# octavian-ganea/equidock_public

Measured on AMD Instinct MI355X. Metric: protein-pairs/sec (fwd+bwd) per IEGMN stack, higher is better.
Workload: dtype f32; 1 GPU; B: DB5.5-sized batch of 8 pairs x (200,200) residues, k=10, 8-layer IEGMN hdim 64, 50 heads, fp32; pairs_per_gpu=8, nodes_per_gpu=3200, edges_per_gpu=32000, layers=8, parallelism=dp1, weights=PyTorch default init (seed 0), ROT key/query x40 (SURVEY.md section 8c), svd_guard_pairs=0, launch_mode=hipGraph replay

## Files before the change

equidock_public_amd/_lib.py:

```python
import ctypes as C
import os

import torch

HERE = os.path.dirname(os.path.abspath(__file__))
LIB_PATH = os.path.join(HERE, 'libequidock_hip.so')
if os.environ.get('EQD_EXP_LIBRARY'):
    LIB_PATH = os.environ['EQD_EXP_LIBRARY']

EQD_MAX_SRC = 6
ABI_VERSION = 9
PARAMS_PER_LAYER = 19
GLOBAL_PARAMS = 5

c_float_p = C.POINTER(C.c_float)
c_int_p = C.POINTER(C.c_int32)


class EqdGraph(C.Structure):
    _fields_ = [('n_pairs', C.c_int32), ('n_lig', C.c_int32), ('n_rec', C.c_int32), ('n_nodes', C.c_int32),
                ('n_edges', C.c_int32), ('n_tiles', C.c_int32), ('n_att_items', C.c_int32), ('max_seg', C.c_int32),
                ('seg_off', C.c_void_p), ('src', C.c_void_p), ('dst', C.c_void_p), ('rowptr', C.c_void_p),
                ('csc_ptr', C.c_void_p), ('csc_eid', C.c_void_p), ('tile_node', C.c_void_p),
                ('att_items', C.c_void_p), ('res_id', C.c_void_p), ('mu_r_norm', C.c_void_p), ('he', C.c_void_p),
# ... 60 lines not shown
                ('dln_b', C.c_void_p), ('dW2', C.c_void_p), ('db2', C.c_void_p), ('dWc1', C.c_void_p),
                ('dbc1', C.c_void_p), ('dwc2', C.c_void_p), ('dbc2', C.c_void_p)]


_lib = None
_is_sim = False
profiling = False


class EquidockHipError(RuntimeError):
    pass


def _declare(lib):
    lib.eqd_abi_version.restype = C.c_int
    lib.eqd_last_error.restype = C.c_char_p
    lib.eqd_tile_edges.restype = C.c_int
    lib.eqd_is_simulator.restype = C.c_int
    lib.eqd_model_saved_bytes.restype = C.c_size_t
    lib.eqd_model_scratch_bytes.restype = C.c_size_t
    lib.eqd_atb_partial_bytes.restype = C.c_size_t
    lib.eqd_edge_message_bwd_workspace_bytes.restype = C.c_size_t
    lib.eqd_keypoint_pool_bwd_workspace_bytes.restype = C.c_size_t
    lib.eqd_clash_workspace_bytes.restype = C.c_size_t
    lib.eqd_node_update_bwd_workspace_bytes.restype = C.c_size_t
    lib.eqd_cross_attention_bwd_ds_workspace_bytes.restype = C.c_size_t
    lib.eqd_profile_name.restype = C.c_char_p
    lib.eqd_profile_us.restype = C.c_float
    lib.eqd_tunables_reload.restype = None
    for name in ('eqd_model_layer_state', 'eqd_model_lrelu_signs', 'eqd_model_head_backward', 'eqd_profile_begin', 'eqd_profile_end', 'eqd_profile_mark', 'eqd_ctx_create', 'eqd_ctx_destroy', 'eqd_model_check', 'eqd_model_forward', 'eqd_model_backward', 'eqd_linear', 'eqd_atb',
                 'eqd_edge_message_fwd', 'eqd_edge_message_bwd', 'eqd_edge_message_bwd_kernel_only',
                 'eqd_cross_attention_fwd', 'eqd_cross_attention_fwd_bf16', 'eqd_cross_attention_bwd_bf16',
                 'eqd_cross_attention_bwd', 'eqd_cross_attention_bwd_ds',
           'eqd_keypoint_pool_fwd', 'eqd_keypoint_pool_bwd', 'eqd_kabsch_fwd', 'eqd_kabsch_bwd',
                 'eqd_rigid_apply_fwd', 'eqd_rigid_apply_bwd', 'eqd_pair_losses_fwd', 'eqd_pair_losses_bwd', 'eqd_scalar_loss', 'eqd_pocket_ot_cost',
                 'eqd_pocket_ot_fwd', 'eqd_pocket_ot_bwd', 'eqd_rigid_augment', 'eqd_protein_graph_distances',
                 'eqd_protein_graph_select', 'eqd_protein_graph_edges', 'eqd_clash_iterations', 'eqd_dropout_pack_edges', 'eqd_dropout_draw',
                 'eqd_node_update_fwd', 'eqd_node_update_bwd', 'eqd_selftest_lane_exchanges'):
        getattr(lib, name).restype = C.c_int


EXPORTS = ('eqd_model_layer_state', 'eqd_model_lrelu_signs', 'eqd_model_head_backward', 'eqd_profile_begin', 'eqd_profile_end', 'eqd_profile_mark', 'eqd_profile_name', 'eqd_profile_us', 'eqd_ctx_create', 'eqd_ctx_destroy', 'eqd_abi_version', 'eqd_last_error', 'eqd_tile_edges', 'eqd_is_simulator', 'eqd_model_saved_bytes', 'eqd_model_saved_layout',
           'eqd_model_scratch_bytes', 'eqd_model_check', 'eqd_model_forward', 'eqd_model_backward', 'eqd_linear',
           'eqd_atb_partial_bytes', 'eqd_atb', 'eqd_edge_message_fwd', 'eqd_edge_message_bwd_workspace_bytes',
           'eqd_edge_message_bwd', 'eqd_edge_message_bwd_kernel_only', 'eqd_cross_attention_fwd',
           'eqd_cross_attention_bwd', 'eqd_cross_attention_bwd_ds', 'eqd_cross_attention_bwd_ds_workspace_bytes', 'eqd_cross_attention_fwd_bf16', 'eqd_cross_attention_bwd_bf16',
           'eqd_keypoint_pool_fwd', 'eqd_keypoint_pool_bwd',
           'eqd_keypoint_pool_bwd_workspace_bytes',
           'eqd_kabsch_fwd', 'eqd_kabsch_bwd', 'eqd_rigid_apply_fwd', 'eqd_rigid_apply_bwd', 'eqd_pair_losses_fwd',
           'eqd_pair_losses_bwd', 'eqd_scalar_loss', 'eqd_pocket_ot_cost', 'eqd_pocket_ot_fwd', 'eqd_pocket_ot_bwd',
           'eqd_rigid_augment', 'eqd_protein_graph_distances', 'eqd_protein_graph_select', 'eqd_protein_graph_edges',
           'eqd_clash_workspace_bytes', 'eqd_clash_iterations', 'eqd_dropout_pack_edges', 'eqd_dropout_draw',
           'eqd_tunables_reload', 'eqd_node_update_fwd', 'eqd_node_update_bwd_workspace_bytes', 'eqd_node_update_bwd',
           'eqd_selftest_lane_exchanges', 'eqd_chain_resident_proj_launches', 'eqd_selftest_node_chain_fwd', 'eqd_model_node_state')


def load_library():
    global _lib, _is_sim
    if _lib is not None:
        return _lib
    if not os.path.exists(LIB_PATH):
        raise EquidockHipError(
            f"{LIB_PATH} is missing: build it with `python -m equidock_public_amd.build` (hipcc, gfx950). "
            "There is no CPU fallback for the IEGMN hot path.")
    lib = C.CDLL(LIB_PATH)
    _declare(lib)
    if lib.eqd_abi_version() != ABI_VERSION:
        raise EquidockHipError(f"ABI version mismatch: library {lib.eqd_abi_version()} != {ABI_VERSION}")
    _lib, _is_sim = lib, bool(lib.eqd_is_simulator())
    return _lib


def load_library_for_testing(path):
    global _lib, _is_sim
    lib = C.CDLL(path)
    _declare(lib)
    _lib, _is_sim = lib, bool(lib.eqd_is_simulator())
    return _lib


def unload_for_testing():
    global _lib, _is_sim
    _lib, _is_sim = None, False


tunables_generation = 0


def reload_tunables():
    global tunables_generation
    tunables_generation += 1
    if _lib is not None:
        _lib.eqd_tunables_reload()


def is_simulator():
    return _is_sim


def check(rc):
    if rc != 0:
        raise EquidockHipError(f"libequidock_hip error {rc}: {_lib.eqd_last_error().decode()}")


def require_device(t, what='tensor'):
    if _is_sim:
        if t.is_cuda:
# ... 62 lines not shown
```

equidock_public_amd/csrc/eqd_common.h:

```cpp
#pragma once
#include <hip/hip_runtime.h>
#include <stdint.h>

#include "../../include/equidock_hip.h"

typedef float f32x4 __attribute__((ext_vector_type(4)));
typedef unsigned int u32x4 __attribute__((ext_vector_type(4)));

#define EQD_BLOCK 256
#define EQD_WAVES 4
#define EQD_NEG_BIG (-1.0e30f)

__device__ __forceinline__ f32x4 mfma4(float a, float b, f32x4 c) {
    return __builtin_amdgcn_mfma_f32_16x16x4f32(a, b, c, 0, 0, 0);
}
#ifdef EQD_TRACE
extern __device__ long long eqd_trace_buf[1024];
#define EQD_TR(slot)                                                                          \
    do {                                                                                      \
        const int trs_ = (slot);                                                              \
        if (blockIdx.x == 0 && blockIdx.y == 0 && threadIdx.x == 0 && trs_ < 256) {           \
            eqd_trace_buf[2 * trs_] = clock64();                                              \
            eqd_trace_buf[2 * trs_ + 1] = wall_clock64();                                     \
        }                                                                                     \
// ... 319 lines not shown

struct EqdArena {
    char* base;
    size_t size, off;
    bool ok;
    EqdArena(void* p, size_t n) : base((char*)p), size(n), off(0), ok(true) {}
    template <typename T>
    T* take(size_t count) {
        size_t bytes = eqd_align_up(count * sizeof(T));
        if (base == nullptr || off + bytes > size) {
            ok = false;
            off += bytes;
            return nullptr;
        }
        T* r = (T*)(base + off);
        off += bytes;
        return r;
    }
};

#define EQD_RED_MAXSEG 64
struct EqdRedSeg {
    const float* partial;
    int nparts, pstride, n;
    float* out;
    int cols, cols_valid, ld_out;
};
struct EqdRedArg {
    EqdRedSeg s[EQD_RED_MAXSEG];
    int chain_first[EQD_RED_MAXSEG], chain_len[EQD_RED_MAXSEG];
    int chain_blk0[EQD_RED_MAXSEG];
    int nchains;
};
int eqd_launch_reduce_segments(const EqdRedSeg* segs, int nseg, hipStream_t st);
struct EqdRedList {
    EqdRedSeg seg[512];
    int n;
};

#define EQD_CHAIN_MAXJOBS 8
struct EqdChainJob {
    EqdLinJob lin;
    int src_local[EQD_MAX_SRC];
    int out_local;
    int type;
    float* aux;
    int prefetch_next;
    int next_lin;
};
struct EqdChainArg {
    EqdChainJob j[EQD_CHAIN_MAXJOBS];
    int njobs;
};
int eqd_launch_rowchain(const EqdChainJob* jobs, int njobs, int rows, hipStream_t st, int* partial_rows = nullptr);
size_t eqd_atb_batch_partial_bytes(int rows);
int eqd_atb_tail_wanted(const EqdLinJob* dh0_job, int n_atb_jobs);
int eqd_atb_with_tail(const EqdAtbJob* jobs, int njobs, void* partial, size_t partial_bytes, hipStream_t st,
                      const EqdLinJob* dh0_job, const EqdGraph* g, const float* dh0acc, const float* dh0b, int ld, int d_emb,
                      float* demb, float* emb_partial, EqdRedList* defer);
int eqd_rows_resident(int rows);
int eqd_rowres80_on();
int eqd_chain_carries_proj(int rows);
int eqd_row_tiles(int rows);
int eqd_rowchain_blocks(int rows);

int eqd_launch_vec_reduce(const float* partial, int nparts, int pstride, int n, float* out, hipStream_t st);
int eqd_launch_embed_fwd(const EqdGraph* g, const float* emb, int d_emb, int use_mu, float* h0, int ld, hipStream_t st);
struct EqdRedList;
int eqd_launch_embed_bwd(const EqdGraph* g, const float* dh0, const float* dh0b, int ld, int d_emb, float* demb,
                         float* partial, hipStream_t st, EqdRedList* defer = nullptr);
size_t eqd_embed_bwd_partial_floats(const EqdGraph* g, int d_emb);
struct EqdGatherCall {
    const float *dz, *dxrel, *d_xnew;
    float a;
    float *dP, *dQ, *dx;
    int dz_bf16;
};
struct EqdGatherArgs;
int eqd_gather_plan(const EqdGraph* g, const EqdGatherCall* c, EqdRedList* pending, EqdGatherArgs* GA, EqdRedArg* RA, int* nblk);
int eqd_gather_rest(EqdRedList* pending, hipStream_t st);
int eqd_attention_bwd_gather_fused(const EqdGraph* g, int d, const float* q, const float* k, const float* v, const float* out,
                                   const float* d_out, bool bf16);
int eqd_attention_ds_stride(const EqdGraph* g);
size_t eqd_attention_ds_bytes(const EqdGraph* g);
int eqd_attention_ds_wanted(const EqdGraph* g, int d, bool bf16);
int eqd_launch_seg_start(const EqdGraph* g, int32_t* seg_start, hipStream_t st);
int eqd_attention_fwd_bf16_impl(const EqdGraph* g, int d, const float* q, const float* k, const float* v, float* out,
                                float* lse, hipStream_t stream, bool qkv_bf16);
int eqd_launch_attention_bwd_gather(const EqdGraph* g, int d, const float* q, const float* k, const float* v, const float* out,
                                    const float* lse, const float* d_out, float* dq, float* dk, float* dv, float* delta,
                                    float qk_slope, bool bf16, const EqdGatherCall* gc, EqdRedList* pending, hipStream_t st,
                                    float* ds = nullptr, const int32_t* seg_start = nullptr, bool qkv_bf16 = false);
int eqd_launch_node_gather(const EqdGraph* g, const float* dz, const float* dxrel, const float* d_xnew, float a,
                           float* dP, float* dQ, float* dx, hipStream_t st, EqdRedList* pending = nullptr,
                           bool dz_bf16 = false);
int eqd_launch_ln_act_bwd(const float* y_act, const float* d_out, const float* gamma, int rows, int d, int ld,
                          float slope, float eps, float* dz, float* dgamma, float* dbeta, float* partial,
                          hipStream_t st, EqdRedList* defer = nullptr);
int eqd_edge_message_bwd_impl(const EqdGraph* g, const EqdEdgeParams* p, const float* P, const float* Q, const float* x,
                              const float* d_aggr_msg, const float* d_xnew, float* dP, float* dQ, float* dx,
                              const EqdEdgeGrads* grads, void* workspace, size_t ws_bytes, hipStream_t st,
                              float* part_override, EqdRedList* defer, EqdGatherCall* hold_gather = nullptr);
size_t eqd_edge_bwd_vecp_floats(const EqdGraph* g);
int eqd_edge_attn_fwd(const EqdGraph* g, const EqdEdgeParams* p, const float* P, const float* Q, const float* x,
                      float* aggr_msg, float* x_new, int d_att, const float* q, const float* k, const float* v,
                      float* att_out, float* lse, hipStream_t st);
int eqd_keypoint_pool_fwd_impl(const EqdGraph* g, int n_heads, const float* Wk, const float* Wq, const float* qmean,
// ... 27 lines not shown
```

equidock_public_amd/csrc/eqd_driver.hip:

```cpp
#include "eqd_common.h"

#include <vector>

#include <string.h>

namespace {

enum {
    P_W1 = 0, P_B1, P_LNG, P_LNB, P_W2, P_B2, P_WQ, P_WK, P_WV, P_WN1, P_BN1, P_NLG, P_NLB, P_WN2, P_BN2,
    P_WC1, P_BC1, P_WC2, P_BC2
};
enum { G_EMB = 0, G_WK, G_WQ, G_WM, G_BM };

struct Dims {
    int N, E, B, K, L, d0, dh;
    int d_in(int l) const { return l == 0 ? d0 : dh; }
    int d_att(int l) const { return (d_in(l) + 15) / 16 * 16; }
    int ldw1(int l) const { return 2 * d_in(l) + 27 + 15; }
    int ldwn(int l) const { return d0 + 2 * d_in(l) + dh; }
};

Dims make_dims(const EqdModelDesc* m, const EqdGraph* g) {
    Dims D;
    D.N = g->n_nodes; D.E = g->n_edges; D.B = g->n_pairs; D.K = m->n_heads; D.L = m->n_layers;
// ... 794 lines not shown
            for (int i = 0; i < nj; ++i) jobs[i] = cj[i].lin;
            RC(eqd_linear(jobs, nj, st));
        }
        hipStream_t sat = (cx && m->cross_msgs) ? cx->sa : st;
        if (sat != st) {
            HIPOK(hipEventRecord(cx->fork, st));
            HIPOK(hipStreamWaitEvent(sat, cx->fork, 0));
        }
        EqdEdgeParams ep = edge_params(D, m, l, p, drop);
        ep.aggr_bf16 = Ls.aggr_b;
        ep.xh_save = Ls.xh_e; ep.rstd_save = Ls.rstd_e; ep.zpos_save = Ls.zpos_e;
        if (m->cross_msgs && sat == st && !m->storage_bf16) {
            RC(eqd_edge_attn_fwd(g, &ep, Ls.P, Ls.Q, S.x[l], Ls.aggr_msg, S.x[l + 1], da, Ls.qa, Ls.ka, Ls.va, Ls.aggr_cross,
                                 Ls.lse, st));
        } else {
            if (m->cross_msgs) {
                if (m->storage_bf16 && Ls.qa_b)
                    RC(eqd_attention_fwd_bf16_impl(g, da, (const float*)Ls.qa_b, (const float*)Ls.ka_b, (const float*)Ls.va_b,
                                                   Ls.aggr_cross, Ls.lse, sat, true));
                else if (m->storage_bf16)
                    RC(eqd_cross_attention_fwd_bf16(g, da, Ls.qa, Ls.ka, Ls.va, Ls.aggr_cross, Ls.lse, sat));
                else
                    RC(eqd_cross_attention_fwd(g, da, Ls.qa, Ls.ka, Ls.va, Ls.aggr_cross, Ls.lse, sat));
            } else {
                if (hipMemsetAsync(Ls.aggr_cross, 0, (size_t)N * da * sizeof(float), st) != hipSuccess) return EQD_ERR_LAUNCH;
            }
            if (sat != st) HIPOK(hipEventRecord(cx->join_a, sat));
            RC(eqd_edge_message_fwd(g, &ep, Ls.P, Ls.Q, S.x[l], Ls.aggr_msg, S.x[l + 1], st));
            if (sat != st) HIPOK(hipStreamWaitEvent(st, cx->join_a, 0));
        }
        NodeFwdChain fc;
        fc.N = N; fc.d = d; fc.da = da; fc.d0 = D.d0; fc.dh = D.dh; fc.ldn = D.ldwn(l); fc.ld_a1n = Ls.ld_a1n;
        fc.slope = slope; fc.eps = eps; fc.skip = m->skip_weight_h;
        fc.h = h; fc.aggr_msg = Ls.aggr_msg; fc.aggr_cross = Ls.aggr_cross; fc.h0 = S.h[0];
        fc.Wn1 = p[P_WN1]; fc.Bn1 = p[P_BN1]; fc.ln_g = p[P_NLG]; fc.ln_b = p[P_NLB]; fc.Wn2 = p[P_WN2]; fc.Bn2 = p[P_BN2];
        fc.drop_mul = drop_node(D, drop, l);
        fc.a1n = Ls.a1n; fc.y_act = Ls.y_act; fc.h_out = S.h[l + 1]; fc.a1n_b = Ls.a1n_b; fc.hb_out = S.hb[l + 1];
        fc.next = nullptr; fc.head = nullptr;
        const bool carry_small = d == 64 && D.dh == 64 && D.d0 > 64 && D.d0 <= 80 && da == 64 && m->cross_msgs &&
                                 !m->storage_bf16 && eqd_chain_carries_proj(N);
        proj_in_chain = l + 1 < D.L && D.d_in(l + 1) == 64 && D.dh == 64 && 2 + (m->cross_msgs ? 5 : 2) <= EQD_CHAIN_MAXJOBS &&
                        (((d == 64 || (m->storage_bf16 && eqd_rowres80_on())) && eqd_rows_resident(N)) ||
                         (carry_small && D.d_att(l + 1) == 64));
        head_in_chain = l + 1 == D.L && carry_small;
        NodePre np;
        if (proj_in_chain) {
            np = node_pre(l + 1);
            fc.next = &np;
        } else if (head_in_chain) {
            fc.head = &jm;
        }
        EqdChainJob cj[EQD_CHAIN_MAXJOBS];
        const int nj = node_fwd_chain(fc, cj);
        RC(eqd_launch_rowchain(cj, nj, N, st));
    }
    if (!head_in_chain) RC(eqd_linear(&jm, 1, st));
    const float* H = S.h[D.L];
    const float* Z = S.x[D.L];
    RC(eqd_launch_seg_mean(g, S.hm, S.qmean, st));
    RC(eqd_keypoint_pool_fwd_impl(g, D.K, gp[G_WK], gp[G_WQ], S.qmean, H, Z, S.Y, Y_lig, Y_rec, S.scores, S.klse, S.qp,
                                  S.u, st, S.Yc));
    RC(eqd_kabsch_fwd_impl(D.B, D.K, S.Y, svd_draws, m->svd_seed, S.T, T, b, S.A, svd_status, st, g, lig_out,
                           S.usv));
    return EQD_OK;
}

static int head_backward(const EqdModelDesc* m, const EqdGraph* g, const Dims& D, const Saved& S, const Scratch& W,
                         const float* const* gpar, float* const* ggrad, const EqdDropout* drop, const float* d_lig,
                         const float* d_Ylig, const float* d_Yrec, const float* d_T, const float* d_b, const float* d_h_last,
                         const float* d_x_last, float* dH_L, float* dX_L, hipStream_t st, EqdRedList* defer,
                         std::vector<EqdAtbJob>& wjobs) {
    const int N = D.N, B = D.B, K = D.K;
    const float slope = m->lrelu_slope, eps = m->ln_eps;
    RC(eqd_kabsch_bwd_impl(B, K, S.Y, S.A, S.T, d_T, d_b, d_Ylig, d_Yrec, W.dY, st, g, d_lig, S.usv));
    const float* H = S.h[D.L];
    const float* Z = S.x[D.L];
    int du_chunks = 1;
    RC(eqd_launch_keypoint_bwd(g, K, H, Z, S.scores, S.klse, S.u, W.dY, W.dscores, W.du, W.dHk, dX_L, st, S.Yc, &du_chunks));
    if (d_h_last) RC(eqd_launch_axpy(W.dHk, d_h_last, 1.f, (size_t)N * 64, st));
    if (d_x_last) RC(eqd_launch_axpy(dX_L, d_x_last, 1.f, (size_t)N * 3, st));
    RC(eqd_launch_head_u_bwd(g, K, gpar[G_WK], gpar[G_WQ], S.qmean, S.qp, du_chunks > 1 ? W.dscores : W.du, ggrad[G_WK],
                             ggrad[G_WQ], W.dqm_part, st, W.head_part, defer, du_chunks));
    RC(eqd_launch_qmean_bwd(g, K, W.dqm_part, W.dhm, st));
    if (drop) {
        const size_t n = (size_t)N * 64;
        hipLaunchKernelGGL(k_mul_inplace, dim3((unsigned)((n + 255) / 256 > 2048 ? 2048 : (n + 255) / 256)), dim3(256), 0, st,
                           W.dhm, drop->head, n);
        RC(eqd_check_launch("k_mul_inplace"));
    }
    EqdLinJob j = lin_job(N, D.dh, dH_L, D.dh, slope, eps);
    lin_src(j, 0, W.dhm, 64, 64, gpar[G_WM], 1, D.dh, S.hm);
    j.nsrc = 1; j.R = W.dHk; j.ldr = 64; j.beta = 1.f;
    RC(eqd_linear(&j, 1, st));
    wjobs.push_back(atb_job(W.dhm, 64, 64, H, D.dh, D.dh, N, ggrad[G_WM], D.dh, ggrad[G_BM], slope, S.hm));
    return EQD_OK;
}

extern "C" int eqd_model_head_backward(const EqdModelDesc* m, const EqdGraph* g, const float* const* params,
                                       const EqdDropout* drop, const float* d_lig, const float* d_Ylig, const float* d_Yrec,
                                       const float* d_T, const float* d_b, float* grad_flat, const int64_t* grad_offsets,
                                       const void* saved, size_t saved_bytes, void* scratch, size_t scratch_bytes,
                                       float* d_h_L, float* d_x_L, void* stream) {
    RC(eqd_model_check(m, g));
    if (!params || !grad_flat || !grad_offsets || !saved || !scratch || !d_h_L || !d_x_L) {
        eqd_set_error("eqd_model_head_backward: NULL argument");
        return EQD_ERR_NULL;
    }
// ... 432 lines not shown
```

equidock_public_amd/csrc/eqd_node_kernels.hip:

```cpp
#include "eqd_common.h"
#include "eqd_linear_inl.h"
#include "eqd_rowwave_inl.h"
#include "eqd_rowres_inl.h"
#include "eqd_rowres80_inl.h"
#include "eqd_chainres_inl.h"
#include "eqd_gather_inl.h"

#include <atomic>
#include <mutex>
#include <vector>

#include <stdarg.h>
#include <stdio.h>
#include <stdlib.h>
#include <string.h>

static thread_local char g_err[512] = "";

void eqd_set_error(const char* fmt, ...) {
    va_list ap;
    va_start(ap, fmt);
    vsnprintf(g_err, sizeof(g_err), fmt, ap);
    va_end(ap);
}
namespace {
struct EqdTunable {
    char name[32];
    char value[32];
    bool set;
};
EqdTunable g_tun[32];
int g_tun_n = 0;
std::mutex g_tun_mu;
}
const char* eqd_tunable(const char* name) {
    static thread_local char ring[8][sizeof(((EqdTunable*)0)->value)];
    static thread_local int ring_at = 0;
    std::lock_guard<std::mutex> lk(g_tun_mu);
    const EqdTunable* hit = nullptr;
    for (int i = 0; i < g_tun_n && !hit; ++i)
        if (strcmp(g_tun[i].name, name) == 0) hit = &g_tun[i];
    if (!hit) {
        const char* v = getenv(name);
        if (g_tun_n >= 32 || strlen(name) >= sizeof(g_tun[0].name) || (v && strlen(v) >= sizeof(g_tun[0].value))) return v;
        EqdTunable& t = g_tun[g_tun_n++];
        snprintf(t.name, sizeof(t.name), "%s", name);
        t.set = v != nullptr;
        snprintf(t.value, sizeof(t.value), "%s", v ? v : "");
        hit = &t;
    }
    if (!hit->set) return nullptr;
    char* out = ring[ring_at];
    ring_at = (ring_at + 1) & 7;
    memcpy(out, hit->value, sizeof(hit->value));
    return out;
}
extern "C" void eqd_tunables_reload(void) {
    std::lock_guard<std::mutex> lk(g_tun_mu);
// ... 829 lines not shown
    return !(f && f[0] == '0' && f[1] == 0);
}
static int chain_resident_proj_on() {
    const char* f = eqd_tunable("EQD_CHAIN_RESIDENT_PROJ");
    return chain_resident_on() && !(f && f[0] == '0' && f[1] == 0);
}
static bool cr_fwd_rows_ok(int rows) {
    const char* oc = eqd_tunable("EQD_ROWCHAIN_OCC");
    return chain_resident_on() && !(oc && oc[0]) && rows > 0 && eqd_row_tiles(rows) == 1 && eqd_rowchain_blocks(rows) <= eqd_num_cus();
}
int eqd_chain_carries_proj(int rows) { return chain_resident_proj_on() && cr_fwd_rows_ok(rows) && rw_mode(rows) == 0; }
static bool crf_pack(const EqdChainJob* jobs, int njobs, int rows, ChainResFwdArg& A, int& np) {
    if (njobs < 2 || !cr_fwd_rows_ok(rows)) return false;
    np = njobs - 2;
    if (np != 0 && !((np == 1 || np == 5) && chain_resident_proj_on())) return false;
    const EqdChainJob &C0 = jobs[0], &C1 = jobs[1];
    const EqdLinJob &J0 = C0.lin, &J1 = C1.lin;
    if (C0.type != 0 || C1.type != 0 || J0.bf16 || J1.bf16 || J0.rows != rows || J1.rows != rows) return false;
    if (J0.M != 64 || J0.nsrc != 4 || C0.out_local != 0 || !J0.ln_g || !J0.ln_b || J0.R) return false;
    for (int s = 0; s < 4; ++s) {
        const EqdLinSrc& S = J0.s[s];
        if (!S.X || !S.W || S.mask || S.w_cs != 1 || C0.src_local[s] >= 0) return false;
        if (s < 3 ? S.K != 64 : (S.K <= 64 || S.K > 80)) return false;
    }
    if (J1.M != 64 || J1.nsrc != 1 || C1.src_local[0] != 0 || J1.ln_g || J1.mul || J1.pre_ln) return false;
    if (np == 0 ? C1.out_local >= 0 : C1.out_local < 0) return false;
    if (J1.s[0].K != 64 || !J1.s[0].W || J1.s[0].mask || J1.s[0].w_cs != 1) return false;
    memset(&A, 0, sizeof(A));
    A.rows = rows; A.K3 = J0.s[3].K;
    for (int s = 0; s < 4; ++s) A.s[s] = CrfSrc{J0.s[s].X, J0.s[s].W, J0.s[s].ldx, J0.s[s].w_rs};
    A.act0 = J0.act; A.slope0 = J0.slope; A.ln_eps = J0.ln_eps; A.alpha0 = J0.alpha; A.beta0 = J0.beta;
    A.bias0 = J0.bias; A.ln_g = J0.ln_g; A.ln_b = J0.ln_b; A.mul0 = J0.mul; A.ld_mul0 = J0.ld_mul;
    A.pre_ln = J0.pre_ln; A.ld_pre = J0.ld_pre; A.Y0 = J0.Y; A.ldy0 = J0.ldy; A.Yb0 = J0.Yb; A.ldyb0 = J0.ldyb;
    A.W1 = J1.s[0].W; A.w1_rs = J1.s[0].w_rs; A.bias1 = J1.bias; A.R1 = J1.R; A.ldr1 = J1.ldr;
    A.act1 = J1.act; A.slope1 = J1.slope; A.alpha1 = J1.alpha; A.beta1 = J1.beta;
    A.Y1 = J1.Y; A.ldy1 = J1.ldy; A.Yb1 = J1.Yb; A.ldyb1 = J1.ldyb;
    for (int j = 0; j < np; ++j) {
        const EqdChainJob& C = jobs[2 + j];
        const EqdLinJob& J = C.lin;
        if (C.type != 0 || J.bf16 || J.rows != rows || J.M != 64 || J.nsrc != 1 || C.src_local[0] != C1.out_local ||
            C.out_local >= 0 || J.s[0].K != 64 || !J.s[0].W || J.s[0].w_cs != 1 || J.s[0].mask || J.ln_g || J.ln_b || J.R ||
            J.pre_ln || J.Yb || J.pad_to != 0 || !J.Y || (J.mul && np != 1))
            return false;
        A.p[j] = CrfProj{J.s[0].W, J.bias, J.Y, J.s[0].w_rs, J.ldy, J.act, J.slope, J.alpha, J.beta};
        if (J.mul) { A.pmul = J.mul; A.ld_pmul = J.ld_mul; }
    }
    return true;
}
static std::atomic<long long> g_chain_resident_launches{0};
extern "C" long long eqd_chain_resident_launches(void) { return g_chain_resident_launches.load(); }
static std::atomic<long long> g_chain_resident_proj_launches{0};
extern "C" long long eqd_chain_resident_proj_launches(void) { return g_chain_resident_proj_launches.load(); }

static int chain_resident_bwd_on() {
    const char* f = eqd_tunable("EQD_CHAIN_RESIDENT_BWD");
    return chain_resident_on() && !(f && f[0] == '0' && f[1] == 0);
}
static bool crb_pack(const EqdChainJob* jobs, int njobs, int rows, ChainResBwdArg& A) {
    if (!chain_resident_bwd_on() || (njobs != 5 && njobs != 6) || rows <= 0 || eqd_row_tiles(rows) != 1 ||
        eqd_rowchain_blocks(rows) > eqd_num_cus())
        return false;
    const bool dh = njobs == 6;
    auto plain = [&](const EqdChainJob& C, int nsrc) {
        const EqdLinJob& J = C.lin;
        if (C.type != 0 || J.bf16 || J.rows != rows || J.M != 64 || J.nsrc != nsrc || J.act || J.bias || J.ln_g || J.ln_b ||
            J.pre_ln || J.mul || J.pad_to != 0 || J.Yb)
            return false;
        for (int s = 0; s < nsrc; ++s)
            if (!J.s[s].W || J.s[s].mask || J.s[s].K != 64 || J.s[s].w_rs != 1) return false;
        return true;
    };
    auto src = [](const EqdLinSrc& S) { return CrbSrc{S.X, S.W, S.ldx, S.w_cs}; };
    auto out = [](const EqdLinJob& J) { return CrbOut{J.Y, J.R, J.ldy, J.ldr, J.alpha, J.beta}; };
    memset(&A, 0, sizeof(A));
    A.rows = rows;
    int at = 0;
    if (dh) {
        const EqdChainJob& C = jobs[at++];
        if (!plain(C, 6) || C.out_local != 2 || !C.lin.Y || !C.lin.R) return false;
        for (int s = 0; s < 6; ++s) {
            if (!C.lin.s[s].X || C.src_local[s] >= 0) return false;
            A.dh[s] = src(C.lin.s[s]);
        }
        A.dho = out(C.lin);
    }
    {
        const EqdChainJob& C = jobs[at++];
        if (!plain(C, 1) || C.out_local != 0 || C.lin.Y || C.lin.R) return false;
        if (dh ? C.src_local[0] != 2 : (C.src_local[0] >= 0 || !C.lin.s[0].X)) return false;
        A.a = src(C.lin.s[0]);
        A.a_alpha = C.lin.alpha;
        A.a_beta = C.lin.beta;
    }
    {
        const EqdChainJob& C = jobs[at++];
        const EqdLinJob& J = C.lin;
        if (C.type != 1 || J.bf16 || J.rows != rows || J.M != 64 || C.src_local[0] != 0 || C.out_local != 1 || !J.s[0].X ||
            !J.ln_g || !J.Y || !C.aux)
            return false;
        A.y_act = J.s[0].X; A.ld_y = J.s[0].ldx;
        A.ln_g = J.ln_g;
        A.mul = J.mul; A.ld_mul = J.ld_mul;
        A.dz = J.Y; A.ld_dz = J.ldy;
        A.aux = C.aux;
        A.slope = J.slope; A.ln_eps = J.ln_eps;
    }
    for (int j = 0; j < 3; ++j) {
        const EqdChainJob& C = jobs[at++];
        if (!plain(C, 1) || C.src_local[0] != 1 || C.out_local >= 0 || !C.lin.Y) return false;
        if (C.lin.R && !(dh && j == 2 && C.lin.R == C.lin.Y && C.lin.ldr == C.lin.ldy)) return false;
        A.x[j] = src(C.lin.s[0]);
        A.xo[j] = out(C.lin);
        if (j > 0 && (A.x[j].W != A.x[j - 1].W + 64 || A.x[j].wcs != A.x[j - 1].wcs)) return false;
    }
    return true;
}
static std::atomic<long long> g_chain_resident_bwd_launches{0};
extern "C" long long eqd_chain_resident_bwd_launches(void) { return g_chain_resident_bwd_launches.load(); }

int eqd_launch_rowchain(const EqdChainJob* jobs, int njobs, int rows, hipStream_t st, int* partial_rows) {
    if (njobs <= 0 || njobs > EQD_CHAIN_MAXJOBS) {
        eqd_set_error("eqd_launch_rowchain: %d jobs (1..%d)", njobs, EQD_CHAIN_MAXJOBS);
        return EQD_ERR_SHAPE;
    }
    if (rows <= 0) return EQD_OK;
    EqdChainArg arg;
    memset(&arg, 0, sizeof(arg));
    for (int i = 0; i < njobs; ++i) {
        arg.j[i] = jobs[i];
        const EqdLinJob& J = jobs[i].lin;
        if (J.M < 4 || J.M > 80 || J.rows != rows) {
            eqd_set_error("eqd_launch_rowchain: job %d has M=%d rows=%d (chain rows %d)", i, J.M, J.rows, rows);
            return EQD_ERR_SHAPE;
        }
        if (jobs[i].type == 0)
            if (int e = lin_check_sources(J)) return e;
        for (int s = 0; s < J.nsrc; ++s)
            if (jobs[i].src_local[s] >= 0 && (J.s[s].K > 80 || jobs[i].src_local[s] >= LIN_LOCALS)) {
                eqd_set_error("eqd_launch_rowchain: LDS-resident source wider than %d or tile index >= %d", 80, LIN_LOCALS);
                return EQD_ERR_SHAPE;
            }
    }
    arg.njobs = njobs;
    chain_links(arg, jobs, njobs);
    for (int i = 0; i < njobs; ++i)
        if (jobs[i].out_local >= LIN_LOCALS) {
            eqd_set_error("eqd_launch_rowchain: LDS tile index %d >= %d", jobs[i].out_local, LIN_LOCALS);
            return EQD_ERR_SHAPE;
        }
    const bool bf = njobs > 0 && jobs[0].lin.bf16;
    if (!rw_eligible(jobs, njobs, rows) && rw80_eligible(jobs, njobs, rows)) {
        if (partial_rows) *partial_rows = rr_blocks(rows);
        const int tps = rr_tiles_per_wg(rows);
        hipLaunchKernelGGL(k_rowres80, dim3(rr_blocks(rows)), dim3(64 * RR_WAVES), 0, st, arg, tps);
        return eqd_check_launch("k_rowres");
    }
    if (rw_eligible(jobs, njobs, rows)) {
        if (partial_rows) *partial_rows = rw_launch_blocks(jobs, njobs, rows);
        return launch_rowwave(arg, rows, bf, st);
    }
    if (partial_rows) *partial_rows = eqd_rowchain_blocks(rows);
    {
        ChainResFwdArg farg;
        int np = 0;
        if (crf_pack(jobs, njobs, rows, farg, np)) {
            const dim3 grid(eqd_rowchain_blocks(rows));
            if (np == 5) hipLaunchKernelGGL(HIP_KERNEL_NAME(k_rowchain_res_fwd<5>), grid, dim3(EQD_BLOCK), 0, st, farg);
            else if (np == 1) hipLaunchKernelGGL(HIP_KERNEL_NAME(k_rowchain_res_fwd<1>), grid, dim3(EQD_BLOCK), 0, st, farg);
            else hipLaunchKernelGGL(HIP_KERNEL_NAME(k_rowchain_res_fwd<0>), grid, dim3(EQD_BLOCK), 0, st, farg);
            g_chain_resident_launches.fetch_add(1);
            if (np) g_chain_resident_proj_launches.fetch_add(1);
            return eqd_check_launch("k_rowchain");
        }
        ChainResBwdArg barg;
        const char* oc = eqd_tunable("EQD_ROWCHAIN_OCC");
        if (!(oc && oc[0]) && crb_pack(jobs, njobs, rows, barg)) {
            if (njobs == 6) hipLaunchKernelGGL(HIP_KERNEL_NAME(k_rowchain_res_bwd<true>), dim3(eqd_rowchain_blocks(rows)), dim3(EQD_BLOCK), 0, st, barg);
            else hipLaunchKernelGGL(HIP_KERNEL_NAME(k_rowchain_res_bwd<false>), dim3(eqd_rowchain_blocks(rows)), dim3(EQD_BLOCK), 0, st, barg);
            g_chain_resident_bwd_launches.fetch_add(1);
            return eqd_check_launch("k_rowchain");
        }
    }
    if (eqd_row_tiles(rows) == 2) {
        if (bf) hipLaunchKernelGGL(HIP_KERNEL_NAME(k_rowchain<2, true, 1>), dim3(eqd_rowchain_blocks(rows)), dim3(EQD_BLOCK), 0, st, arg);
        else hipLaunchKernelGGL(HIP_KERNEL_NAME(k_rowchain<2, false, 1>), dim3(eqd_rowchain_blocks(rows)), dim3(EQD_BLOCK), 0, st, arg);
    } else {
        const char* oc = eqd_tunable("EQD_ROWCHAIN_OCC");
        const bool one = oc && (oc[0] == '1' || oc[0] == '2') && oc[1] == 0 ? oc[0] == '1' : eqd_rowchain_blocks(rows) <= eqd_num_cus();
        if (bf && one) hipLaunchKernelGGL(HIP_KERNEL_NAME(k_rowchain<1, true, 1>), dim3(eqd_rowchain_blocks(rows)), dim3(EQD_BLOCK), 0, st, arg);
        else if (bf) hipLaunchKernelGGL(HIP_KERNEL_NAME(k_rowchain<1, true, 2>), dim3(eqd_rowchain_blocks(rows)), dim3(EQD_BLOCK), 0, st, arg);
        else if (one) hipLaunchKernelGGL(HIP_KERNEL_NAME(k_rowchain<1, false, 1>), dim3(eqd_rowchain_blocks(rows)), dim3(EQD_BLOCK), 0, st, arg);
        else hipLaunchKernelGGL(HIP_KERNEL_NAME(k_rowchain<1, false, 2>), dim3(eqd_rowchain_blocks(rows)), dim3(EQD_BLOCK), 0, st, arg);
    }
    return eqd_check_launch("k_rowchain");
}

extern "C" int eqd_linear(const EqdLinJob* jobs, int njobs, void* stream) {
    if (!jobs || njobs <= 0) {
        eqd_set_error("eqd_linear: no jobs");
        return EQD_ERR_NULL;
    }
    hipStream_t st = (hipStream_t)stream;
    if (njobs <= EQD_CHAIN_MAXJOBS) {
        EqdChainArg carg;
        memset(&carg, 0, sizeof(carg));
        bool ok = true;
        for (int i = 0; i < njobs && ok; ++i) {
            EqdChainJob& C = carg.j[i];
            C.lin = jobs[i];
            for (int s = 0; s < EQD_MAX_SRC; ++s) C.src_local[s] = -1;
            C.out_local = -1;
            ok = (jobs[i].Y != nullptr || jobs[i].Yb != nullptr) && jobs[i].rows == jobs[0].rows;
        }
        if (ok && !rw_eligible(carg.j, njobs, jobs[0].rows) && rw80_eligible(carg.j, njobs, jobs[0].rows)) {
            for (int i = 0; i < njobs; ++i)
                if (int e = lin_check_sources(jobs[i])) return e;
            carg.njobs = njobs;
            const int rows80 = jobs[0].rows, tps = rr_tiles_per_wg(rows80);
            hipLaunchKernelGGL(k_rowres80, dim3(rr_blocks(rows80)), dim3(64 * RR_WAVES), 0, st, carg, tps);
            return eqd_check_launch("k_rowres");
        }
        if (ok && rw_eligible(carg.j, njobs, jobs[0].rows)) {
            for (int i = 0; i < njobs; ++i)
                if (int e = lin_check_sources(jobs[i])) return e;
// ... 1003 lines not shown
```

include/equidock_hip.h:

```cpp
#ifndef EQUIDOCK_HIP_H
#define EQUIDOCK_HIP_H

#include <stddef.h>
#include <stdint.h>

#ifdef __cplusplus
extern "C" {
#endif

#define EQD_ABI_VERSION 9
#define EQD_TILE_EDGES 32
#define EQD_ATT_BLOCK 32
#define EQD_MAX_SRC 6
#define EQD_PARAMS_PER_LAYER 19
#define EQD_GLOBAL_PARAMS 5

enum {
    EQD_OK = 0,
    EQD_ERR_NULL = 1,
    EQD_ERR_SHAPE = 2,
    EQD_ERR_UNSUPPORTED = 3,
    EQD_ERR_WORKSPACE = 4,
    EQD_ERR_LAUNCH = 5
};

int eqd_abi_version(void);
const char* eqd_last_error(void);
int eqd_tile_edges(void);
int eqd_is_simulator(void);
void eqd_tunables_reload(void);
long long eqd_chain_resident_launches(void);
long long eqd_chain_resident_bwd_launches(void);
typedef struct EqdNodeChainBwdTest {
    int32_t rows, with_dh, d0;
    float skip_weight_h, slope, ln_eps;
    const float* dh_X[6];
    const float* dh_W[6];
    int32_t dh_wcs[6];
    const float* dH_above;
    float* dH;
    const float* Wn2;
    const float* Wn1;
    const float* y_act;
    const float* ln_g;
    const float* drop_mul;
    float* dz;
    float* ln_part;
    float* d_aggr_msg;
    float* d_aggr_cross;
    float* dh0acc;
} EqdNodeChainBwdTest;
int eqd_selftest_node_chain_bwd(const EqdNodeChainBwdTest* t, int* partial_rows , void* stream);
long long eqd_chain_resident_proj_launches(void);
typedef struct EqdNodeChainFwdTest {
    int32_t rows, d0, form;
    float skip_weight_h, slope, ln_eps;
    const float* h; const float* aggr_msg; const float* aggr_cross; const float* h0;
    const float* Wn1; const float* Bn1; const float* ln_g; const float* ln_b; const float* Wn2; const float* Bn2;
    const float* drop_mul;
    float* a1n; float* y_act; float* h_out;
    const float* W1; const float* B1; const float* WQ; const float* WK; const float* WV;
    float* P; float* Q; float* qa; float* ka; float* va;
    const float* WM; const float* BM; const float* head_mul ; float* hm;
} EqdNodeChainFwdTest;
int eqd_selftest_node_chain_fwd(const EqdNodeChainFwdTest* t, void* stream);
int eqd_selftest_lane_exchanges(const float* in256, int* mismatch, float* out256, void* stream);

int eqd_profile_begin(void* stream, int max_launches);
int eqd_profile_end(void);
int eqd_profile_mark(const char* label);
const char* eqd_profile_name(int i);
float eqd_profile_us(int i);

typedef struct EqdGraph {
    int32_t n_pairs, n_lig, n_rec, n_nodes, n_edges, n_tiles, n_att_items, max_seg;
    const int32_t* seg_off;
    const int32_t* src;
    const int32_t* dst;
    const int32_t* rowptr;
    const int32_t* csc_ptr;
    const int32_t* csc_eid;
    const int32_t* tile_node;
    const int32_t* att_items;
    const int32_t* res_id;
    const float* mu_r_norm;
    const float* he;
    const float* x0;
    const uint16_t* he_bf16;
} EqdGraph;

typedef struct EqdModelDesc {
    int32_t n_layers;
    int32_t d_emb;
    int32_t d_hid;
    int32_t use_mean_node_features;
    int32_t edge_feats;
    int32_t n_heads;
    int32_t cross_msgs, use_dist_in_layers, use_edge_features;
    float skip_weight_h, x_connection_init, lrelu_slope, ln_eps;
    int32_t svd_seed;
    int32_t storage_bf16;
} EqdModelDesc;

typedef struct EqdDropout {
    float p;
    const uint32_t* edge_z1;
// ... 219 lines not shown
```

Measured before the change: 8266 pairs/s.

## Add resident-weight wide rowchain forward kernel for the 69-wide node MLP chain

Adds a specialised forward kernel for the two-job node-update chain where the first linear has M=69 with four sources and the second projects 69 to 64. It stages all weights, including the remainder columns beyond 64, into LDS alongside input tiles, and computes linear, LayerNorm and the second linear in one block with MFMA. This replaces the generic rowchain path for that shape. The kernel runs only when cross messages are enabled and an env tunable does not disable it. It uses a large shared-memory footprint at one block per CU and adds hand-written remainder handling that could hurt occupancy.

```diff
diff --git a/equidock_public_amd/_lib.py b/equidock_public_amd/_lib.py
--- a/equidock_public_amd/_lib.py
+++ b/equidock_public_amd/_lib.py
@@ -136,7 +136,8 @@
            'eqd_rigid_augment', 'eqd_protein_graph_distances', 'eqd_protein_graph_select', 'eqd_protein_graph_edges',
            'eqd_clash_workspace_bytes', 'eqd_clash_iterations', 'eqd_dropout_pack_edges', 'eqd_dropout_draw',
            'eqd_tunables_reload', 'eqd_node_update_fwd', 'eqd_node_update_bwd_workspace_bytes', 'eqd_node_update_bwd',
-           'eqd_selftest_lane_exchanges', 'eqd_chain_resident_proj_launches', 'eqd_selftest_node_chain_fwd', 'eqd_model_node_state')
+           'eqd_selftest_lane_exchanges', 'eqd_chain_resident_proj_launches', 'eqd_selftest_node_chain_fwd', 'eqd_model_node_state',
+           'eqd_chain_resident_wide_launches')
 
 
 def load_library():
diff --git a/equidock_public_amd/csrc/eqd_chainres_wide_inl.h b/equidock_public_amd/csrc/eqd_chainres_wide_inl.h
--- /dev/null
+++ b/equidock_public_amd/csrc/eqd_chainres_wide_inl.h
@@ -0,0 +1,275 @@
+#pragma once
+#include "eqd_chainres_inl.h"
+
+#define CRW_CHUNK (80 * 64)
+#define CRW_REM (128 * 8)
+struct alignas(1024) ChainResWideSmem {
+    float W[4][CRW_CHUNK];
+    float W1[CR_CHUNK];
+    float Wr[4][CRW_REM];
+    float X[4][CR_XTILE];
+    float Xr[4][256];
+};
+struct ChainResWideArg {
+    int rows, M;
+    int act0, ld_mul0, ld_pre, ldy0;
+    int act1, w1_rs, ldy1;
+    float slope0, ln_eps, alpha0, beta0, slope1, alpha1, beta1;
+    CrfSrc s[4];
+    const float *bias0, *ln_g, *ln_b, *mul0;
+    float *pre_ln, *Y0;
+    const float *W1, *bias1;
+    float* Y1;
+};
+
+__device__ __forceinline__ void crw_copy_chunk(const float* Wg, int w_rs, int M, float* img, int wave, int lane) {
+#pragma unroll
+    for (int i = 0; i < 4; ++i) {
+        const int m = 16 * wave + 4 * i + (lane >> 4);
+        glds16(Wg + (size_t)m * w_rs + 4 * ((lane & 15) ^ (m & 15)), &img[64 * (16 * wave + 4 * i)]);
+    }
+    const int r = 64 + 4 * wave + (lane >> 4);
+    const int m = r < M ? r : M - 1;
+    glds16(Wg + (size_t)m * w_rs + 4 * ((lane & 15) ^ (r & 15)), &img[64 * (64 + 4 * wave)]);
+}
+__device__ __forceinline__ void crw_copy_rem(const float* Wg, int w_rs, int M, int K, float* img, int wave, int lane) {
+    const int r = 32 * wave + (lane >> 1);
+    const int m = r < M ? r : M - 1;
+    glds16(Wg + (size_t)m * w_rs + ((lane & 1) ? K - 4 : 64), &img[256 * wave]);
+}
+__device__ __forceinline__ f32x4 crw_rem_frag(const float* __restrict__ img, int r, int g) {
+    const f32x4 v = *(const f32x4*)&img[8 * r + (g == 1 ? 4 : 0)];
+    f32x4 o;
+    o[0] = g == 0 ? v[0] : (g == 1 ? v[3] : 0.f);
+    o[1] = g == 0 ? v[1] : 0.f;
+    o[2] = g == 0 ? v[2] : 0.f;
+    o[3] = g == 0 ? v[3] : 0.f;
+    return o;
+}
+__device__ __forceinline__ void crw_mma(f32x4 (&acc)[2], f32x4 (&acc2)[2], const float* __restrict__ Wi,
+                                        const float* __restrict__ Xi, int wave, bool own1, int l15, int g) {
+    f32x4 a[4], a4[4], b[4];
+#pragma unroll
+    for (int q = 0; q < 4; ++q) a[q] = *(const f32x4*)&Wi[cr_at(16 * wave + l15, 4 * q + g)];
+#pragma unroll
+    for (int q = 0; q < 4; ++q) b[q] = *(const f32x4*)&Xi[cr_at(l15, 4 * q + g)];
+    if (own1) {
+#pragma unroll
+        for (int q = 0; q < 4; ++q) a4[q] = *(const f32x4*)&Wi[cr_at(64 + l15, 4 * q + g)];
+    }
+#ifndef EQD_HOSTSIM
+    __builtin_amdgcn_sched_barrier(0);
+#endif
+#pragma unroll
+    for (int q = 0; q < 4; ++q) {
+        acc[0] = mfma4(a[q][0], b[q][0], acc[0]);
+        acc2[0] = mfma4(a[q][1], b[q][1], acc2[0]);
+        acc[0] = mfma4(a[q][2], b[q][2], acc[0]);
+        acc2[0] = mfma4(a[q][3], b[q][3], acc2[0]);
+    }
+    if (own1) {
+#pragma unroll
+        for (int q = 0; q < 4; ++q) {
+            acc[1] = mfma4(a4[q][0], b[q][0], acc[1]);
+            acc2[1] = mfma4(a4[q][1], b[q][1], acc2[1]);
+            acc[1] = mfma4(a4[q][2], b[q][2], acc[1]);
+            acc2[1] = mfma4(a4[q][3], b[q][3], acc2[1]);
+        }
+    }
+    keep_after_wait(acc[0]);
+    keep_after_wait(acc2[0]);
+    keep_after_wait(acc[1]);
+    keep_after_wait(acc2[1]);
+}
+__device__ __forceinline__ void crw_mma_rem(f32x4 (&acc)[2], f32x4 (&acc2)[2], const float* __restrict__ Wr, const f32x4 b,
+                                            int wave, bool own1, int l15, int g) {
+    const f32x4 a = crw_rem_frag(Wr, 16 * wave + l15, g);
+    acc[0] = mfma4(a[0], b[0], acc[0]);
+    acc2[0] = mfma4(a[1], b[1], acc2[0]);
+    acc[0] = mfma4(a[2], b[2], acc[0]);
+    acc2[0] = mfma4(a[3], b[3], acc2[0]);
+    if (own1) {
+        const f32x4 a4 = crw_rem_frag(Wr, 64 + l15, g);
+        acc[1] = mfma4(a4[0], b[0], acc[1]);
+        acc2[1] = mfma4(a4[1], b[1], acc2[1]);
+        acc[1] = mfma4(a4[2], b[2], acc[1]);
+        acc2[1] = mfma4(a4[3], b[3], acc2[1]);
+    }
+}
+
+__global__ __launch_bounds__(EQD_BLOCK, 1) void k_rowchain_res_fwd_wide(ChainResWideArg A) {
+    __shared__ ChainResWideSmem S;
+    __shared__ __attribute__((aligned(16))) float Lt[16 * LIN_S];
+    __shared__ float stat[EQD_WAVES][16];
+    const int t = threadIdx.x, lane = t & 63, wave = t >> 6, l15 = lane & 15, g = lane >> 4;
+    const int row0 = (int)blockIdx.x * 16, rows = A.rows, M = A.M;
+    for (int i = t; i < 16 * LIN_S; i += EQD_BLOCK) Lt[i] = 0.f;
+    const int mbn = (M + 15) >> 4;
+    const int mbs[2] = {wave, wave + 4};
+    const bool own[2] = {wave < mbn, wave + 4 < mbn};
+    const int rowi = row0 + l15;
+    const bool rv = rowi < rows;
+    const int rowe = rv ? rowi : rows - 1;
+    f32x4 bias[2], lg[2], lb[2], mulr[2], bias1;
+    int nf[2];
+#pragma unroll
+    for (int i = 0; i < 2; ++i) {
+        const int f0 = 16 * mbs[i] + 4 * g;
+        nf[i] = own[i] ? M - f0 : 0;
+        const float* const bp = A.bias0 ? A.bias0 : A.ln_g;
+        const float* const mp = A.mul0 ? A.mul0 + (size_t)rowe * A.ld_mul0 : A.ln_g;
+        bias[i] = ld4u_raw(bp + f0, nf[i], bp);
+        lg[i] = ld4u_raw(A.ln_g + f0, nf[i], A.ln_g);
+        lb[i] = ld4u_raw(A.ln_b + f0, nf[i], A.ln_b);
+        mulr[i] = ld4u_raw(mp + f0, nf[i], mp);
+    }
+    bias1 = *(const EQD_GAS f4v*)((A.bias1 ? A.bias1 : A.ln_g) + 16 * wave + 4 * g);
+    {
+        const int r = 4 * wave + (lane >> 4);
+        const int c = 4 * ((lane & 15) ^ (r & 15));
+        int row = row0 + r;
+        row = row < rows ? row : rows - 1;
+#pragma unroll
+        for (int s = 0; s < 4; ++s) glds16(A.s[s].X + (size_t)row * A.s[s].ldx + c, &S.X[s][256 * wave]);
+        const float* const xp = wave == 0 ? A.s[0].X : (wave == 1 ? A.s[2].X : A.s[3].X);
+        const int xl = wave == 0 ? A.s[0].ldx : (wave == 1 ? A.s[2].ldx : A.s[3].ldx);
+        int rr = row0 + ((lane >> 1) & 15);
+        rr = rr < rows ? rr : rows - 1;
+        glds16(xp + (size_t)rr * xl + ((lane & 1) ? M - 4 : 64), S.Xr[wave]);
+    }
+    crw_copy_chunk(A.s[0].W, A.s[0].w_rs, M, S.W[0], wave, lane);
+    crw_copy_rem(A.s[0].W, A.s[0].w_rs, M, M, S.Wr[0], wave, lane);
+    crw_copy_chunk(A.s[1].W, A.s[1].w_rs, M, S.W[1], wave, lane);
+    crw_copy_chunk(A.s[2].W, A.s[2].w_rs, M, S.W[2], wave, lane);
+    crw_copy_rem(A.s[2].W, A.s[2].w_rs, M, M, S.Wr[1], wave, lane);
+    crw_copy_chunk(A.s[3].W, A.s[3].w_rs, M, S.W[3], wave, lane);
+    crw_copy_rem(A.s[3].W, A.s[3].w_rs, M, M, S.Wr[2], wave, lane);
+    cr_copy_chunk(A.W1, A.w1_rs, S.W1, wave, lane);
+    crw_copy_rem(A.W1, A.w1_rs, 64, M, S.Wr[3], wave, lane);
+    f32x4 acc[2] = {f4zero(), f4zero()}, acc2[2] = {f4zero(), f4zero()};
+    const bool own1 = own[1];
+    vm_wait<22>();
+    lds_barrier();
+    crw_mma(acc, acc2, S.W[0], S.X[0], wave, own1, l15, g);
+    crw_mma_rem(acc, acc2, S.Wr[0], crw_rem_frag(S.Xr[0], l15, g), wave, own1, l15, g);
+    vm_wait<17>();
+    lds_barrier();
+    crw_mma(acc, acc2, S.W[1], S.X[1], wave, own1, l15, g);
+    vm_wait<11>();
+    lds_barrier();
+    crw_mma(acc, acc2, S.W[2], S.X[2], wave, own1, l15, g);
+    crw_mma_rem(acc, acc2, S.Wr[1], crw_rem_frag(S.Xr[1], l15, g), wave, own1, l15, g);
+    vm_wait<5>();
+    lds_barrier();
+    crw_mma(acc, acc2, S.W[3], S.X[3], wave, own1, l15, g);
+    crw_mma_rem(acc, acc2, S.Wr[2], crw_rem_frag(S.Xr[2], l15, g), wave, own1, l15, g);
+    vm_wait<0>();
+#pragma unroll
+    for (int i = 0; i < 2; ++i) {
+        keep_after_wait(bias[i]); keep_after_wait(lg[i]); keep_after_wait(lb[i]); keep_after_wait(mulr[i]);
+    }
+    keep_after_wait(bias1);
+    if (!A.bias0) bias[0] = bias[1] = f4zero();
+    if (!A.bias1) bias1 = f4zero();
+    {
+        const float slope = A.slope0;
+        float4 bs[2], lgv[2], lbv[2];
+#pragma unroll
+        for (int i = 0; i < 2; ++i) {
+            bs[i] = ld4u_fix(bias[i], nf[i]);
+            lgv[i] = ld4u_fix(lg[i], nf[i]);
+            lbv[i] = ld4u_fix(lb[i], nf[i]);
+        }
+        float v[2][4];
+#pragma unroll
+        for (int i = 0; i < 2; ++i) {
+            const float bb[4] = {bs[i].x, bs[i].y, bs[i].z, bs[i].w};
+#pragma unroll
+            for (int r = 0; r < 4; ++r) {
+                float y = (acc[i][r] + acc2[i][r]) + bb[r];
+                if (A.act0) y = lrelu(y, slope);
+                v[i][r] = r < nf[i] ? y : 0.f;
+            }
+        }
+        if (A.mul0) {
+#pragma unroll
+            for (int i = 0; i < 2; ++i) {
+                const float4 mm = ld4u_fix(mulr[i], nf[i]);
+                v[i][0] *= mm.x; v[i][1] *= mm.y; v[i][2] *= mm.z; v[i][3] *= mm.w;
+            }
+        }
+        const float invM = 1.f / (float)M;
+        float s1 = 0.f;
+#pragma unroll
+        for (int i = 0; i < 2; ++i)
+#pragma unroll
+            for (int r = 0; r < 4; ++r) s1 += v[i][r];
+        s1 = group_sum(s1);
+        if (g == 0) stat[wave][l15] = s1;
+        __syncthreads();
+        const float mean = (stat[0][l15] + stat[1][l15] + stat[2][l15] + stat[3][l15]) * invM;
+        float q = 0.f;
+#pragma unroll
+        for (int i = 0; i < 2; ++i)
+#pragma unroll
+            for (int r = 0; r < 4; ++r) {
+                const float dlt = r < nf[i] ? v[i][r] - mean : 0.f;
+                q += dlt * dlt;
+            }
+        q = group_sum(q);
+        __syncthreads();
+        if (g == 0) stat[wave][l15] = q;
+        __syncthreads();
+        const float rstd = 1.f / sqrtf((stat[0][l15] + stat[1][l15] + stat[2][l15] + stat[3][l15]) * invM + A.ln_eps);
+#pragma unroll
+        for (int i = 0; i < 2; ++i) {
+            const float gg[4] = {lgv[i].x, lgv[i].y, lgv[i].z, lgv[i].w};
+            const float be[4] = {lbv[i].x, lbv[i].y, lbv[i].z, lbv[i].w};
+#pragma unroll
+            for (int r = 0; r < 4; ++r)
+                if (r < nf[i]) {
+                    const int f = 16 * mbs[i] + 4 * g + r;
+                    if (A.pre_ln && rv) ((EQD_GAS float*)A.pre_ln)[(size_t)rowi * A.ld_pre + f] = v[i][r];
+                    v[i][r] = (v[i][r] - mean) * rstd * gg[r] + be[r];
+                }
+        }
+        const float alpha = A.alpha0, beta = A.beta0;
+#pragma unroll
+        for (int i = 0; i < 2; ++i) {
+            const int f0 = 16 * mbs[i] + 4 * g;
+#pragma unroll
+            for (int r = 0; r < 4; ++r) {
+                const float y = alpha * v[i][r] + beta * 0.f;
+                if (r < nf[i]) {
+                    if (A.Y0 && rv) ((EQD_GAS float*)A.Y0)[(size_t)rowi * A.ldy0 + f0 + r] = y;
+                    Lt[l15 * LIN_S + f0 + r] = y;
+                }
+            }
+        }
+    }
+    __syncthreads();
+    {
+        f32x4 c = f4zero(), c2 = f4zero();
+        cr_mma<true>(c, c2, S.W1, Lt, wave, l15, g);
+        const f32x4 a = crw_rem_frag(S.Wr[3], 16 * wave + l15, g);
+        const f32x4 b = *(const f32x4*)&Lt[l15 * LIN_S + 64 + 4 * g];
+        c = mfma4(a[0], b[0], c);
+        c2 = mfma4(a[1], b[1], c2);
+        c = mfma4(a[2], b[2], c);
+        c2 = mfma4(a[3], b[3], c2);
+        const float slope = A.slope1;
+        const int f0 = 16 * wave + 4 * g;
+        float v[4];
+#pragma unroll
+        for (int r = 0; r < 4; ++r) {
+            float y = (c[r] + c2[r]) + bias1[r];
+            if (A.act1) y = lrelu(y, slope);
+            v[r] = y;
+        }
+        const float alpha = A.alpha1, beta = A.beta1;
+        f32x4 yv;
+#pragma unroll
+        for (int r = 0; r < 4; ++r) yv[r] = alpha * v[r] + beta * 0.f;
+        if (A.Y1 && rv) *(EQD_GAS f4v*)&A.Y1[(size_t)rowi * A.ldy1 + f0] = yv;
+    }
+}
diff --git a/equidock_public_amd/csrc/eqd_common.h b/equidock_public_amd/csrc/eqd_common.h
--- a/equidock_public_amd/csrc/eqd_common.h
+++ b/equidock_public_amd/csrc/eqd_common.h
@@ -395,7 +395,8 @@
     EqdChainJob j[EQD_CHAIN_MAXJOBS];
     int njobs;
 };
-int eqd_launch_rowchain(const EqdChainJob* jobs, int njobs, int rows, hipStream_t st, int* partial_rows = nullptr);
+int eqd_launch_rowchain(const EqdChainJob* jobs, int njobs, int rows, hipStream_t st, int* partial_rows = nullptr,
+                        bool wide_ok = true);
 size_t eqd_atb_batch_partial_bytes(int rows);
 int eqd_atb_tail_wanted(const EqdLinJob* dh0_job, int n_atb_jobs);
 int eqd_atb_with_tail(const EqdAtbJob* jobs, int njobs, void* partial, size_t partial_bytes, hipStream_t st,
diff --git a/equidock_public_amd/csrc/eqd_driver.hip b/equidock_public_amd/csrc/eqd_driver.hip
--- a/equidock_public_amd/csrc/eqd_driver.hip
+++ b/equidock_public_amd/csrc/eqd_driver.hip
@@ -870,7 +870,7 @@
         }
         EqdChainJob cj[EQD_CHAIN_MAXJOBS];
         const int nj = node_fwd_chain(fc, cj);
-        RC(eqd_launch_rowchain(cj, nj, N, st));
+        RC(eqd_launch_rowchain(cj, nj, N, st, nullptr, m->cross_msgs != 0));
     }
     if (!head_in_chain) RC(eqd_linear(&jm, 1, st));
     const float* H = S.h[D.L];
diff --git a/equidock_public_amd/csrc/eqd_node_kernels.hip b/equidock_public_amd/csrc/eqd_node_kernels.hip
--- a/equidock_public_amd/csrc/eqd_node_kernels.hip
+++ b/equidock_public_amd/csrc/eqd_node_kernels.hip
@@ -4,6 +4,7 @@
 #include "eqd_rowres_inl.h"
 #include "eqd_rowres80_inl.h"
 #include "eqd_chainres_inl.h"
+#include "eqd_chainres_wide_inl.h"
 #include "eqd_gather_inl.h"
 
 #include <atomic>
@@ -939,6 +940,39 @@
 static std::atomic<long long> g_chain_resident_proj_launches{0};
 extern "C" long long eqd_chain_resident_proj_launches(void) { return g_chain_resident_proj_launches.load(); }
 
+static int chain_resident_wide_on() {
+    const char* f = eqd_tunable("EQD_CHAIN_RESIDENT_WIDE");
+    return chain_resident_on() && !(f && f[0] == '0' && f[1] == 0);
+}
+static bool crw_pack(const EqdChainJob* jobs, int njobs, int rows, ChainResWideArg& A) {
+    if (njobs != 2 || !chain_resident_wide_on() || !cr_fwd_rows_ok(rows) || rw_mode(rows) != 0) return false;
+    const EqdChainJob &C0 = jobs[0], &C1 = jobs[1];
+    const EqdLinJob &J0 = C0.lin, &J1 = C1.lin;
+    if (C0.type != 0 || C1.type != 0 || J0.bf16 || J1.bf16 || J0.rows != rows || J1.rows != rows) return false;
+    if (J0.M != 69 || J0.nsrc != 4 || C0.out_local != 0 || !J0.ln_g || !J0.ln_b || J0.R || J0.Yb || J0.pad_to != 0) return false;
+    for (int s = 0; s < 4; ++s) {
+        const EqdLinSrc& S = J0.s[s];
+        if (!S.X || !S.W || S.mask || S.w_cs != 1 || C0.src_local[s] >= 0) return false;
+        if (S.K != (s == 1 ? 64 : 69) || S.ldx < S.K) return false;
+    }
+    if (J1.M != 64 || J1.nsrc != 1 || C1.src_local[0] != 0 || C1.out_local >= 0 || J1.ln_g || J1.ln_b || J1.mul || J1.pre_ln ||
+        J1.R || J1.Yb || J1.pad_to != 0 || !J1.Y)
+        return false;
+    if (J1.s[0].K != 69 || !J1.s[0].W || J1.s[0].mask || J1.s[0].w_cs != 1) return false;
+    memset(&A, 0, sizeof(A));
+    A.rows = rows; A.M = J0.M;
+    for (int s = 0; s < 4; ++s) A.s[s] = CrfSrc{J0.s[s].X, J0.s[s].W, J0.s[s].ldx, J0.s[s].w_rs};
+    A.act0 = J0.act; A.slope0 = J0.slope; A.ln_eps = J0.ln_eps; A.alpha0 = J0.alpha; A.beta0 = J0.beta;
+    A.bias0 = J0.bias; A.ln_g = J0.ln_g; A.ln_b = J0.ln_b; A.mul0 = J0.mul; A.ld_mul0 = J0.ld_mul;
+    A.pre_ln = J0.pre_ln; A.ld_pre = J0.ld_pre; A.Y0 = J0.Y; A.ldy0 = J0.ldy;
+    A.W1 = J1.s[0].W; A.w1_rs = J1.s[0].w_rs; A.bias1 = J1.bias;
+    A.act1 = J1.act; A.slope1 = J1.slope; A.alpha1 = J1.alpha; A.beta1 = J1.beta;
+    A.Y1 = J1.Y; A.ldy1 = J1.ldy;
+    return true;
+}
+static std::atomic<long long> g_chain_resident_wide_launches{0};
+extern "C" long long eqd_chain_resident_wide_launches(void) { return g_chain_resident_wide_launches.load(); }
+
 static int chain_resident_bwd_on() {
     const char* f = eqd_tunable("EQD_CHAIN_RESIDENT_BWD");
     return chain_resident_on() && !(f && f[0] == '0' && f[1] == 0);
@@ -1005,7 +1039,7 @@
 static std::atomic<long long> g_chain_resident_bwd_launches{0};
 extern "C" long long eqd_chain_resident_bwd_launches(void) { return g_chain_resident_bwd_launches.load(); }
 
-int eqd_launch_rowchain(const EqdChainJob* jobs, int njobs, int rows, hipStream_t st, int* partial_rows) {
+int eqd_launch_rowchain(const EqdChainJob* jobs, int njobs, int rows, hipStream_t st, int* partial_rows, bool wide_ok) {
     if (njobs <= 0 || njobs > EQD_CHAIN_MAXJOBS) {
         eqd_set_error("eqd_launch_rowchain: %d jobs (1..%d)", njobs, EQD_CHAIN_MAXJOBS);
         return EQD_ERR_SHAPE;
@@ -1057,6 +1091,12 @@
             else hipLaunchKernelGGL(HIP_KERNEL_NAME(k_rowchain_res_fwd<0>), grid, dim3(EQD_BLOCK), 0, st, farg);
             g_chain_resident_launches.fetch_add(1);
             if (np) g_chain_resident_proj_launches.fetch_add(1);
+            return eqd_check_launch("k_rowchain");
+        }
+        ChainResWideArg warg;
+        if (wide_ok && crw_pack(jobs, njobs, rows, warg)) {
+            hipLaunchKernelGGL(k_rowchain_res_fwd_wide, dim3(eqd_rowchain_blocks(rows)), dim3(EQD_BLOCK), 0, st, warg);
+            g_chain_resident_wide_launches.fetch_add(1);
             return eqd_check_launch("k_rowchain");
         }
         ChainResBwdArg barg;
diff --git a/include/equidock_hip.h b/include/equidock_hip.h
--- a/include/equidock_hip.h
+++ b/include/equidock_hip.h
@@ -52,6 +52,7 @@
 } EqdNodeChainBwdTest;
 int eqd_selftest_node_chain_bwd(const EqdNodeChainBwdTest* t, int* partial_rows , void* stream);
 long long eqd_chain_resident_proj_launches(void);
+long long eqd_chain_resident_wide_launches(void);
 typedef struct EqdNodeChainFwdTest {
     int32_t rows, d0, form;
     float skip_weight_h, slope, ln_eps;
```

Result: faster. 8394 pairs/s (median of 6 runs) (+1.6%).
